# bdina9/qat-vit

Hardware: AMD Instinct MI355X
Metric: images/sec QAT student step (fwd+bwd+allreduce) (higher is better)
Workload: dtype f32 (emulated: int8 MFMA for grid x grid products; forward float operands as fp16 hi+lo pairs; backward gradients as ONE fp16 plane scaled per tensor - 2^-12 per element, <= 4e-4 relative L2 per stage against the fp32 reference, bf16-pair fallback on overflow; fp32 / exact-integer accumulate)

## Files before the change

### qat-vit_amd/csrc/elt.hip

```cpp
#include <stdlib.h>

#include "qv_common.h"
#include "qv_kernels.h"
#include "qv_qparams.h"

namespace qv {

typedef __bf16 bf16x4 __attribute__((ext_vector_type(4)));
typedef __bf16 bf16x8 __attribute__((ext_vector_type(8)));

struct QP { float s, inv, zp, on; };
__device__ inline QP load_qp(const float* qp) { return QP{qp[0], qp[1], qp[2], qp[3]}; }
__device__ inline float fqv(float x, const QP& q, float fqmin, float fqmax, bool& in) {
    const float t = rintf(x * q.inv) + q.zp;
    in = (t >= fqmin && t <= fqmax) || q.on == 0.f;
    const float y = (fminf(fmaxf(t, fqmin), fqmax) - q.zp) * q.s;
    return q.on != 0.f ? y : x;
}
__device__ inline float fqi(float x, const QP& q, float fqmin, float fqmax) {
    return fminf(fmaxf(rintf(x * q.inv) + q.zp, fqmin), fqmax) - q.zp;
}

__device__ inline void store_split4(__bf16* hi, __bf16* lo, int64_t off, float a, float b, float c, float d) {
    uint2 h, l;
    split_pair(a, b, h.x, l.x);
    split_pair(c, d, h.y, l.y);
    *reinterpret_cast<uint2*>(hi + off) = h;
    *reinterpret_cast<uint2*>(lo + off) = l;
}

__device__ inline void store_f16x4(__bf16* plane, int64_t off, float a, float b, float c, float d, float mul, float& am) {
    am = fmaxf(fmaxf(am, fmaxf(fabsf(a), fabsf(b))), fmaxf(fabsf(c), fabsf(d)));
    *reinterpret_cast<uint2*>(plane + off) = make_uint2(pk_f16(a * mul, b * mul), pk_f16(c * mul, d * mul));
}
__device__ inline void amax_publish(uint32_t* amax, float am, int lane) {
    am = wave_max(am);
    if (lane == 0) atomicMax(amax + (blockIdx.x & (kDyAmaxSlots - 1)) * kDyAmaxStride, __builtin_bit_cast(uint32_t, am));
}

static inline int rows_grid(int64_t rows) {
    int64_t b = (rows + 3) / 4;
    return (int)(b < 1 ? 1 : (b > 2048 ? 2048 : b));
}
static inline int flat_grid(int64_t n4) {
    int64_t b = (n4 + 255) / 256;
    return (int)(b < 1 ? 1 : (b > 4096 ? 4096 : b));
}

__global__ __launch_bounds__(256) void k_img_patches(const float* __restrict__ img, __bf16* __restrict__ out, const float* __restrict__ qp,
                                                     int qmin, int qmax, int B, int C, int H, int W, int P, int8_t* __restrict__ out8, int center) {
    const QP q = load_qp(qp);
    const int gw = W / P, gh = H / P, K = C * P * P;
    const int64_t n8 = (int64_t)B * gh * gw * K / 8;
    for (int64_t e8 = blockIdx.x * (int64_t)blockDim.x + threadIdx.x; e8 < n8; e8 += (int64_t)gridDim.x * blockDim.x) {
        const int64_t e = e8 * 8;
        const int col = (int)(e % K);
        const int64_t prow = e / K;
        const int px = (int)(prow % gw), py = (int)((prow / gw) % gh), b = (int)(prow / ((int64_t)gw * gh));
        const int j = col % P, i = (col / P) % P, c = col / (P * P);
        const float* src = img + (((int64_t)b * C + c) * H + py * P + i) * W + px * P + j;
        const float4 a = reinterpret_cast<const float4*>(src)[0], bb = reinterpret_cast<const float4*>(src)[1];
        bf16x8 o;
        o[0] = (__bf16)fqi(a.x, q, qmin, qmax); o[1] = (__bf16)fqi(a.y, q, qmin, qmax);
        o[2] = (__bf16)fqi(a.z, q, qmin, qmax); o[3] = (__bf16)fqi(a.w, q, qmin, qmax);
        o[4] = (__bf16)fqi(bb.x, q, qmin, qmax); o[5] = (__bf16)fqi(bb.y, q, qmin, qmax);
        o[6] = (__bf16)fqi(bb.z, q, qmin, qmax); o[7] = (__bf16)fqi(bb.w, q, qmin, qmax);
        if (out) *reinterpret_cast<bf16x8*>(out + e) = o;
        if (out8) {
            const float sh = q.zp - (float)center;
            signed char c8[8];
#pragma unroll
            for (int t = 0; t < 8; ++t) c8[t] = (signed char)((float)o[t] + sh);
            uint2 pk;
            __builtin_memcpy(&pk, c8, 8);
            *reinterpret_cast<uint2*>(out8 + e) = pk;
        }
    }
}

constexpr int kMaxV = 3;
__device__ inline void pin4(float4& v) { asm volatile("" : "+v"(v.x), "+v"(v.y), "+v"(v.z), "+v"(v.w)); }
template <int MODE, int NV>
__global__ __launch_bounds__(256) void k_resid_fq_lnstats(const float* __restrict__ x_prev, const float* __restrict__ Y, const float* __restrict__ qpY,
                                                          int qmin, int qmax, const float* __restrict__ cls, const float* __restrict__ pos,
                                                          float* __restrict__ x_new, float* __restrict__ mean, float* __restrict__ rstd,
                                                          const float* __restrict__ gamma, const float* __restrict__ beta, float eps,
                                                          uint32_t* __restrict__ stats, int stat_slots, int64_t M, int D, int T,
                                                          unsigned long long* __restrict__ maskbits, const QpLate late) {
    __shared__ float sQp[4];
    QP q;
    if (late.stats) { const float4 r = qp_late_resolve(late, sQp); q = QP{r.x, r.y, r.z, r.w}; }
    else q = load_qp(qpY);
    const int lane = threadIdx.x & 63;
    bool act[NV];
    int cc[NV];
    float4 g[NV], bb[NV];
#pragma unroll
    for (int j = 0; j < NV; ++j) {
        const int c = lane * 4 + 256 * j;
        act[j] = c < D;
        cc[j] = act[j] ? c : 0;
        g[j] = *reinterpret_cast<const float4*>(gamma + cc[j]);
        bb[j] = *reinterpret_cast<const float4*>(beta + cc[j]);
    }
    float mn = INFINITY, mx = -INFINITY;
    for (int64_t row = (int64_t)blockIdx.x * 4 + (threadIdx.x >> 6); row < M; row += (int64_t)gridDim.x * 4) {
        const int t = (int)(row % T);
        const int64_t b = row / T;
        const bool is_cls = MODE == 0 && t == 0;
        const float* bsrc = MODE == 0 ? pos + (int64_t)t * D : x_prev + row * D;
        const float* ysrc = MODE == 0 ? (is_cls ? cls : Y + (b * (T - 1) + (t - 1)) * D) : MODE == 1 ? Y + row * D : bsrc;
        float4 yr[NV], base[NV], v[NV];
#pragma unroll
        for (int j = 0; j < NV; ++j) {
            base[j] = *reinterpret_cast<const float4*>(bsrc + cc[j]);
            yr[j] = *reinterpret_cast<const float4*>(ysrc + cc[j]);
        }
#pragma unroll
        for (int j = 0; j < NV; ++j) { pin4(base[j]); pin4(yr[j]); }
        float s = 0.f;
        unsigned long long mb[NV][4];
#pragma unroll
        for (int j = 0; j < NV; ++j) {
            bool i0, i1, i2, i3;
            float4 y = make_float4(fqv(yr[j].x, q, qmin, qmax, i0), fqv(yr[j].y, q, qmin, qmax, i1), fqv(yr[j].z, q, qmin, qmax, i2),
                                   fqv(yr[j].w, q, qmin, qmax, i3));
            if (is_cls) y = yr[j];
            if (MODE == 2) y = make_float4(0.f, 0.f, 0.f, 0.f);
            if (MODE == 1) {
                mb[j][0] = __ballot(act[j] && i0); mb[j][1] = __ballot(act[j] && i1);
                mb[j][2] = __ballot(act[j] && i2); mb[j][3] = __ballot(act[j] && i3);
            }
            v[j] = make_float4(base[j].x + y.x, base[j].y + y.y, base[j].z + y.z, base[j].w + y.w);
            if (act[j]) s += (v[j].x + v[j].y) + (v[j].z + v[j].w);
        }
#pragma unroll
        for (int j = 0; j < NV; ++j)
            if (MODE != 2 && act[j]) *reinterpret_cast<float4*>(x_new + row * D + cc[j]) = v[j];
        const float mu = wave_sum(s) / (float)D;
        float qq = 0.f;
#pragma unroll
        for (int j = 0; j < NV; ++j) {
            v[j].x -= mu; v[j].y -= mu; v[j].z -= mu; v[j].w -= mu;
            if (act[j]) qq += (v[j].x * v[j].x + v[j].y * v[j].y) + (v[j].z * v[j].z + v[j].w * v[j].w);
        }
        const float rs = rsqrtf(wave_sum(qq) / (float)D + eps);
        if (lane == 0) { mean[row] = mu; rstd[row] = rs; }
        if (MODE == 1 && maskbits && lane < 4) {
#pragma unroll
            for (int j = 0; j < NV; ++j)
                maskbits[(row * NV + j) * 4 + lane] = lane == 0 ? mb[j][0] : lane == 1 ? mb[j][1] : lane == 2 ? mb[j][2] : mb[j][3];
        }
#pragma unroll
        for (int j = 0; j < NV; ++j) {
            if (act[j]) {
                const float o0 = v[j].x * rs * g[j].x + bb[j].x, o1 = v[j].y * rs * g[j].y + bb[j].y, o2 = v[j].z * rs * g[j].z + bb[j].z,
                            o3 = v[j].w * rs * g[j].w + bb[j].w;
                mn = fminf(fminf(mn, o0), fminf(o1, fminf(o2, o3)));
                mx = fmaxf(fmaxf(mx, o0), fmaxf(o1, fmaxf(o2, o3)));
            }
        }
    }
    mn = wave_min(mn);
    mx = wave_max(mx);
    __shared__ float smn[4], smx[4];
    if (lane == 0) { smn[threadIdx.x >> 6] = mn; smx[threadIdx.x >> 6] = mx; }
    __syncthreads();
    const float bmn = fminf(fminf(smn[0], smn[1]), fminf(smn[2], smn[3])), bmx = fmaxf(fmaxf(smx[0], smx[1]), fmaxf(smx[2], smx[3]));
    if (threadIdx.x == 0) stat_atomic(stats, stat_slots, bmn, bmx);
}

__global__ __launch_bounds__(256) void k_ln_apply_quant(const float* __restrict__ x, const float* __restrict__ mean, const float* __restrict__ rstd,
                                                        const float* __restrict__ gamma, const float* __restrict__ beta, const float* __restrict__ qp,
                                                        int qmin, int qmax, __bf16* __restrict__ out, int64_t M, int D,
                                                        int8_t* __restrict__ out8, int center, int out_f16, const QpLate late) {
    __shared__ float sQp[4];
    QP q;
    if (late.stats) { const float4 r = qp_late_resolve(late, sQp); q = QP{r.x, r.y, r.z, r.w}; }
    else q = load_qp(qp);
    const int d4 = D / 4;
    const int64_t n4 = M * d4;
    for (int64_t i = blockIdx.x * (int64_t)blockDim.x + threadIdx.x; i < n4; i += (int64_t)gridDim.x * blockDim.x) {
        const int64_t row = i / d4;
        const int c = (int)(i % d4) * 4;
        const float mu = mean[row], rs = rstd[row];
        const float4 v = *reinterpret_cast<const float4*>(x + row * D + c);
        const float4 g = *reinterpret_cast<const float4*>(gamma + c), b = *reinterpret_cast<const float4*>(beta + c);
        bf16x4 o;
        o[0] = (__bf16)fqi((v.x - mu) * rs * g.x + b.x, q, qmin, qmax);
        o[1] = (__bf16)fqi((v.y - mu) * rs * g.y + b.y, q, qmin, qmax);
        o[2] = (__bf16)fqi((v.z - mu) * rs * g.z + b.z, q, qmin, qmax);
        o[3] = (__bf16)fqi((v.w - mu) * rs * g.w + b.w, q, qmin, qmax);
        if (out && out_f16) *reinterpret_cast<uint2*>(out + row * D + c) = make_uint2(pk_f16((float)o[0], (float)o[1]), pk_f16((float)o[2], (float)o[3]));
        else if (out) *reinterpret_cast<bf16x4*>(out + row * D + c) = o;
        if (out8) {
            const float sh = q.zp - (float)center;
            char4 o8 = make_char4((signed char)((float)o[0] + sh), (signed char)((float)o[1] + sh), (signed char)((float)o[2] + sh),
                                  (signed char)((float)o[3] + sh));
            *reinterpret_cast<char4*>(out8 + row * D + c) = o8;
        }
    }
}

template <int NV>
__global__ __launch_bounds__(256) void k_ln_quant8(const float* __restrict__ x, const float* __restrict__ gamma, const float* __restrict__ beta, float eps,
                                                   const float* __restrict__ qp, int qmin, int qmax, int center, int8_t* __restrict__ out8,
                                                   float* __restrict__ mean, float* __restrict__ rstd, int64_t nrows, int64_t row_stride, int D) {
    const QP q = load_qp(qp);
    const int lane = threadIdx.x & 63;
    bool act[NV];
    int cc[NV];
    float4 g[NV], bb[NV];
#pragma unroll
    for (int j = 0; j < NV; ++j) {
        const int c = lane * 4 + 256 * j;
        act[j] = c < D;
        cc[j] = act[j] ? c : 0;
        g[j] = *reinterpret_cast<const float4*>(gamma + cc[j]);
        bb[j] = *reinterpret_cast<const float4*>(beta + cc[j]);
    }
    const float sh = q.zp - (float)center;
    for (int64_t i = (int64_t)blockIdx.x * 4 + (threadIdx.x >> 6); i < nrows; i += (int64_t)gridDim.x * 4) {
        const int64_t row = i * row_stride;
        float4 v[NV];
#pragma unroll
        for (int j = 0; j < NV; ++j) v[j] = *reinterpret_cast<const float4*>(x + row * D + cc[j]);
#pragma unroll
        for (int j = 0; j < NV; ++j) pin4(v[j]);
        float s = 0.f;
#pragma unroll
        for (int j = 0; j < NV; ++j)
            if (act[j]) s += (v[j].x + v[j].y) + (v[j].z + v[j].w);
        const float mu = wave_sum(s) / (float)D;
        float qq = 0.f;
        float4 cv[NV];
#pragma unroll
        for (int j = 0; j < NV; ++j) {
            cv[j] = make_float4(v[j].x - mu, v[j].y - mu, v[j].z - mu, v[j].w - mu);
            if (act[j]) qq += (cv[j].x * cv[j].x + cv[j].y * cv[j].y) + (cv[j].z * cv[j].z + cv[j].w * cv[j].w);
        }
        const float rs = rsqrtf(wave_sum(qq) / (float)D + eps);
        if (mean && lane == 0) { mean[row] = mu; rstd[row] = rs; }
        if (out8) {
#pragma unroll
            for (int j = 0; j < NV; ++j) {
                if (act[j]) {
                    const char4 o = make_char4((signed char)(fqi(cv[j].x * rs * g[j].x + bb[j].x, q, qmin, qmax) + sh),
                                               (signed char)(fqi(cv[j].y * rs * g[j].y + bb[j].y, q, qmin, qmax) + sh),
                                               (signed char)(fqi(cv[j].z * rs * g[j].z + bb[j].z, q, qmin, qmax) + sh),
                                               (signed char)(fqi(cv[j].w * rs * g[j].w + bb[j].w, q, qmin, qmax) + sh));
                    *reinterpret_cast<char4*>(out8 + row * D + cc[j]) = o;
                }
            }
        }
    }
}

__global__ __launch_bounds__(256) void k_cls_rows(const float* __restrict__ cls, const float* __restrict__ pos, float* __restrict__ x, int B, int T, int D) {
    const int64_t n = (int64_t)B * D;
    for (int64_t i = blockIdx.x * (int64_t)blockDim.x + threadIdx.x; i < n; i += (int64_t)gridDim.x * blockDim.x) {
        const int b = (int)(i / D), c = (int)(i % D);
        x[(int64_t)b * T * D + c] = cls[c] + pos[c];
    }
}

__device__ inline float gelu(float x) { return gelu_fwd(x); }
__device__ inline float dgelu(float x) { return gelu_bwd(x); }

template <int GELU_BWD, bool O16 = false>
__global__ __launch_bounds__(256) void k_mask_bwd(const float* __restrict__ d, const float* __restrict__ Y, const float* __restrict__ qp,
                                                  int qmin, int qmax, const float* __restrict__ col_scale, int ncols4,
                                                  __bf16* __restrict__ dst_hi, __bf16* __restrict__ dst_lo, int64_t n4,
                                                  const float* __restrict__ o16_mul, uint32_t* __restrict__ o16_amax) {
    const QP q = load_qp(qp);
    float mul = 1.f, am = 0.f;
    if constexpr (O16) mul = *o16_mul;
    for (int64_t i = blockIdx.x * (int64_t)blockDim.x + threadIdx.x; i < n4; i += (int64_t)gridDim.x * blockDim.x) {
        const float4 v = reinterpret_cast<const float4*>(Y)[i];
        const float4 g = reinterpret_cast<const float4*>(d)[i];
        const float in4[4] = {v.x, v.y, v.z, v.w}, g4[4] = {g.x, g.y, g.z, g.w};
        float cs[4] = {1.f, 1.f, 1.f, 1.f};
        if (col_scale) {
            const float4 c = reinterpret_cast<const float4*>(col_scale)[i % ncols4];
// ... 263 lines not shown
        if (t == 0) *reinterpret_cast<float4*>(dcls + c) = acc;
    }
}

__device__ inline void wquant_body(const float* __restrict__ W, const float* __restrict__ qp, int per_channel, int qmin, int qmax,
                                   __bf16* __restrict__ wq, __bf16* __restrict__ wqT, int N, int K, int bx, int by,
                                   int8_t* __restrict__ w8 = nullptr, int32_t* __restrict__ wsum = nullptr, _Float16* __restrict__ w16 = nullptr,
                                   int8_t* __restrict__ w8f = nullptr, int64_t wT16_gap = 0,
                                   bool wT16_frag = false) {
    __shared__ float tile[32][33];
    const int tx = threadIdx.x & 31, ty = threadIdx.x >> 5;
    const int n0 = by * 32, k0 = bx * 32;
#pragma unroll
    for (int i = 0; i < 4; ++i) {
        const int n = n0 + ty + 8 * i, k = k0 + tx;
        float v = 0.f;
        if (n < N && k < K) {
            const QP q = load_qp(qp + 4 * (per_channel ? n : 0));
            v = q.on != 0.f ? fqi(W[(int64_t)n * K + k], q, qmin, qmax) : W[(int64_t)n * K + k];
            wq[(int64_t)n * K + k] = (__bf16)v;
            if (w8) w8[(int64_t)n * K + k] = (int8_t)v;
            if (w16) w16[(int64_t)n * K + k] = (_Float16)v;
            if (w8f) w8f[w8f_offset(n, k, K)] = (int8_t)v;
        }
        tile[ty + 8 * i][tx] = v;
    }
    __syncthreads();
    if (wsum && threadIdx.x < 32 && n0 + (int)threadIdx.x < N) {
        float sacc = 0.f;
#pragma unroll
        for (int k = 0; k < 32; ++k) sacc += tile[threadIdx.x][k];
        atomicAdd(&wsum[n0 + threadIdx.x], (int)sacc);
    }
    if (wqT) {
        _Float16* const wT16 = wT16_gap ? reinterpret_cast<_Float16*>(reinterpret_cast<char*>(wqT) + wT16_gap) : nullptr;
        char* const wT16f = (wT16_gap && wT16_frag) ? reinterpret_cast<char*>(wqT) + 2 * wT16_gap : nullptr;
#pragma unroll
        for (int i = 0; i < 4; ++i) {
            const int k = k0 + ty + 8 * i, n = n0 + tx;
            if (n < N && k < K) {
                wqT[(int64_t)k * N + n] = (__bf16)tile[tx][ty + 8 * i];
                if (wT16) wT16[(int64_t)k * N + n] = (_Float16)tile[tx][ty + 8 * i];
                if (wT16f) *reinterpret_cast<_Float16*>(wT16f + w8f_offset(k, 2 * n, 2 * N)) = (_Float16)tile[tx][ty + 8 * i];
            }
        }
    }
}
__global__ __launch_bounds__(256) void k_wquant(const float* __restrict__ W, const float* __restrict__ qp, int per_channel, int qmin, int qmax,
                                                __bf16* __restrict__ wq, __bf16* __restrict__ wqT, int N, int K) {
    wquant_body(W, qp, per_channel, qmin, qmax, wq, wqT, N, K, blockIdx.x, blockIdx.y);
}
__global__ __launch_bounds__(256) void k_w_quant_all(const WQuantTab t) {
    int wi = 0;
    while (wi + 1 < t.n && (int)blockIdx.x >= t.blk0[wi + 1]) ++wi;
    const int b = blockIdx.x - t.blk0[wi], kt = (t.K[wi] + 31) / 32;
    wquant_body(t.W[wi], t.qp[wi], t.per_channel, t.qmin, t.qmax, reinterpret_cast<__bf16*>(t.wq[wi]), reinterpret_cast<__bf16*>(t.wqT[wi]), t.N[wi],
                t.K[wi], b % kt, b / kt, reinterpret_cast<int8_t*>(t.w8[wi]), t.wsum[wi], reinterpret_cast<_Float16*>(t.w16[wi]),
                reinterpret_cast<int8_t*>(t.w8f[wi]), t.wT16 ? wT16_gap_bytes(t.N[wi], t.K[wi]) : 0, ((t.wT16f_mask >> wi) & 1ull) != 0);
}
static_assert(sizeof(WQuantTab) <= 4096, "WQuantTab travels as a kernel argument");
__global__ __launch_bounds__(256) void k_w8_fragment_order(const int8_t* __restrict__ B8, int8_t* __restrict__ B8f, int N, int K) {
    const int64_t i = blockIdx.x * (int64_t)blockDim.x + threadIdx.x;
    if (i >= (int64_t)N * K) return;
    B8f[w8f_offset((int)(i / K), (int)(i % K), K)] = B8[i];
}
int launch_w8_fragment_order(const void* B8, void* B8f, int N, int K, hipStream_t st) {
    if (N < 48 || N % 48 != 0 || K % 64 != 0 || !B8 || !B8f) { set_error("w8_fragment_order: need N %% 48 == 0, K %% 64 == 0 (N=%d K=%d)", N, K); return 1; }
    k_w8_fragment_order<<<cdiv((int64_t)N * K, 256), 256, 0, st>>>(reinterpret_cast<const int8_t*>(B8), reinterpret_cast<int8_t*>(B8f), N, K);
    return 0;
}

int launch_img_patches(const float* img, void* out_bf16, const float* qp, int qmin, int qmax, int B, int C, int H, int W, int P, hipStream_t st,
                       void* out8, int center) {
    if (P % 8 != 0 || H % P != 0 || W % P != 0) { set_error("img_patches: patch %d must be a multiple of 8 and divide %dx%d", P, H, W); return 1; }
    const int64_t n8 = (int64_t)B * C * H * W / 8;
    k_img_patches<<<flat_grid(n8), 256, 0, st>>>(img, reinterpret_cast<__bf16*>(out_bf16), qp, qmin, qmax, B, C, H, W, P, reinterpret_cast<int8_t*>(out8),
                                                 center);
    return 0;
}

int launch_resid_fq_lnstats(int mode, const float* x_prev, const float* Y, const float* qpY, int qmin, int qmax, const float* cls, const float* pos,
                            float* x_new, float* mean, float* rstd, const float* gamma, const float* beta, float eps, uint32_t* stats, int stat_slots,
                            int64_t M, int D, int T, hipStream_t st, void* maskbits, const QpLate* late) {
    if (D % 4 != 0 || D > 256 * kMaxV) { set_error("resid_fq_lnstats: D=%d unsupported (need D%%4==0, D<=768)", D); return 1; }
    unsigned long long* mbits = mode != 1 ? nullptr : reinterpret_cast<unsigned long long*>(maskbits);
    const QpLate lt = late ? *late : QpLate{};
#define QV_RESID(MODE_, NV_) k_resid_fq_lnstats<MODE_, NV_><<<rows_grid(M), 256, 0, st>>>(x_prev, Y, qpY, qmin, qmax, cls, pos, x_new, mean, rstd, gamma, beta, eps, stats, stat_slots, M, D, T, mbits, lt)
    const int nv = (D + 255) / 256;
    if (mode == 0) { if (nv == 1) QV_RESID(0, 1); else if (nv == 2) QV_RESID(0, 2); else QV_RESID(0, 3); }
    else if (mode == 1) { if (nv == 1) QV_RESID(1, 1); else if (nv == 2) QV_RESID(1, 2); else QV_RESID(1, 3); }
    else { if (nv == 1) QV_RESID(2, 1); else if (nv == 2) QV_RESID(2, 2); else QV_RESID(2, 3); }
#undef QV_RESID
    return 0;
}

int launch_ln_apply_quant(const float* x, const float* mean, const float* rstd, const float* gamma, const float* beta, const float* qp, int qmin,
                          int qmax, void* out_bf16, int64_t M, int D, hipStream_t st, void* out8, int center, bool out_f16, const QpLate* late) {
    k_ln_apply_quant<<<flat_grid(M * (D / 4)), 256, 0, st>>>(x, mean, rstd, gamma, beta, qp, qmin, qmax, reinterpret_cast<__bf16*>(out_bf16), M, D,
                                                             reinterpret_cast<int8_t*>(out8), center, out_f16 ? 1 : 0, late ? *late : QpLate{});
    return 0;
}

int launch_ln_quant8(const float* x, const float* gamma, const float* beta, float eps, const float* qp, int qmin, int qmax, int center, void* out8,
                     float* mean, float* rstd, int64_t nrows, int64_t row_stride, int D, hipStream_t st) {
    if (D % 4 != 0 || D > 256 * kMaxV) { set_error("ln_quant8: D=%d unsupported (need D%%4==0, D<=768)", D); return 1; }
    const int nv = (D + 255) / 256, grid = rows_grid(nrows);
    int8_t* o = reinterpret_cast<int8_t*>(out8);
    if (nv == 1) k_ln_quant8<1><<<grid, 256, 0, st>>>(x, gamma, beta, eps, qp, qmin, qmax, center, o, mean, rstd, nrows, row_stride, D);
    else if (nv == 2) k_ln_quant8<2><<<grid, 256, 0, st>>>(x, gamma, beta, eps, qp, qmin, qmax, center, o, mean, rstd, nrows, row_stride, D);
    else k_ln_quant8<3><<<grid, 256, 0, st>>>(x, gamma, beta, eps, qp, qmin, qmax, center, o, mean, rstd, nrows, row_stride, D);
    return 0;
}
int launch_cls_rows(const float* cls, const float* pos, float* x, int B, int T, int D, hipStream_t st) {
    k_cls_rows<<<cdiv((int64_t)B * D, 256), 256, 0, st>>>(cls, pos, x, B, T, D);
    return 0;
}

int launch_mask_bwd(int gelu_bwd, const float* d, const float* Y, const float* qp, int qmin, int qmax, const float* col_scale, int ncols,
                    void* dst_hi, void* dst_lo, int64_t n, hipStream_t st, const float* o16_mul, uint32_t* o16_amax) {
    __bf16* h = reinterpret_cast<__bf16*>(dst_hi);
    __bf16* l = reinterpret_cast<__bf16*>(dst_lo);
    if (o16_mul) {
        if (gelu_bwd || !o16_amax) { set_error("mask_bwd: the one-plane form covers the plain mask with o16_amax"); return 1; }
        k_mask_bwd<0, true><<<flat_grid(n / 4), 256, 0, st>>>(d, Y, qp, qmin, qmax, col_scale, ncols / 4, h, l, n / 4, o16_mul, o16_amax);
        return 0;
    }
    if (gelu_bwd) k_mask_bwd<1><<<flat_grid(n / 4), 256, 0, st>>>(d, Y, qp, qmin, qmax, col_scale, ncols / 4, h, l, n / 4, nullptr, nullptr);
    else k_mask_bwd<0><<<flat_grid(n / 4), 256, 0, st>>>(d, Y, qp, qmin, qmax, col_scale, ncols / 4, h, l, n / 4, nullptr, nullptr);
    return 0;
}

int launch_ln_bwd_fq(int acc, const float* dH, const float* x, const float* mean, const float* rstd, const float* gamma, const float* beta,
                     const float* qp, int qmin, int qmax, const float* dx_in, float* dx_out, float* dgamma, float* dbeta, int64_t M, int D, int T,
                     int cls_only, hipStream_t st, const LnBwdNext* next) {
    if (D % 4 != 0 || D > 256 * kMaxV) { set_error("ln_bwd_fq: D=%d unsupported", D); return 1; }
    constexpr int rpw = 16;
    int grid = (int)((M + 8 * rpw - 1) / (8 * rpw));
    if (grid > 4096) grid = 4096;
    if (grid < 1) grid = 1;
    const unsigned long long* nm = next ? reinterpret_cast<const unsigned long long*>(next->maskbits) : nullptr;
    const float* ncs = next ? next->colscale : nullptr;
    __bf16* nh = next ? reinterpret_cast<__bf16*>(next->out_hi) : nullptr;
    __bf16* nl = next ? reinterpret_cast<__bf16*>(next->out_lo) : nullptr;
    const float* m16 = next ? next->o16_mul : nullptr;
    uint32_t* a16 = next ? next->o16_amax : nullptr;
    if (m16 && !a16) { set_error("ln_bwd_fq: o16_mul needs o16_amax"); return 1; }
#define QV_LNB(ACC_, NV_)                                                                                                                          \
    do {                                                                                                                                           \
        if (next && m16) k_ln_bwd_fq<ACC_, NV_, 8, true, true><<<grid, 512, 0, st>>>(dH, 0, x, mean, rstd, gamma, beta, qp, qmin, qmax, dx_in, dx_out, dgamma, dbeta, M, D, T, cls_only, nm, ncs, nh, nl, m16, a16); \
        else if (next) k_ln_bwd_fq<ACC_, NV_, 8, true><<<grid, 512, 0, st>>>(dH, 0, x, mean, rstd, gamma, beta, qp, qmin, qmax, dx_in, dx_out, dgamma, dbeta, M, D, T, cls_only, nm, ncs, nh, nl, nullptr, nullptr); \
        else k_ln_bwd_fq<ACC_, NV_, 8, false><<<grid, 512, 0, st>>>(dH, 0, x, mean, rstd, gamma, beta, qp, qmin, qmax, dx_in, dx_out, dgamma, dbeta, M, D, T, cls_only, nm, ncs, nh, nl, nullptr, nullptr); \
    } while (0)
    const int nv = (D + 255) / 256;
    if (acc) { if (nv == 1) QV_LNB(1, 1); else if (nv == 2) QV_LNB(1, 2); else QV_LNB(1, 3); }
    else { if (nv == 1) QV_LNB(0, 1); else if (nv == 2) QV_LNB(0, 2); else QV_LNB(0, 3); }
#undef QV_LNB
    return 0;
}

int launch_head_fwd(const float* x, const float* mean, const float* rstd, const float* gamma, const float* beta, const float* qp_norm, int qmin,
                    int qmax, const void* wq, const float* w_scale, int w_per_channel, const float* bias, float* hq, float* logits_pre,
                    uint32_t* stats, int stat_slots, int B, int D, int T, int C, hipStream_t st) {
    k_head_fwd<<<B, 256, D * sizeof(float), st>>>(x, mean, rstd, gamma, beta, qp_norm, qmin, qmax, reinterpret_cast<const __bf16*>(wq), w_scale,
                                                   w_per_channel, bias, hq, logits_pre, stats, stat_slots, D, T, C);
    return 0;
}

int launch_logits_fq(const float* pre, const float* qp, int qmin, int qmax, float* out, int n, hipStream_t st) {
    k_logits_fq<<<cdiv(n, 256), 256, 0, st>>>(pre, qp, qmin, qmax, out, n);
    return 0;
}

int launch_head_bwd(const float* dlogits, const float* logits_pre, const float* qp_logits, int qmin, int qmax, const float* hq, const float* qp_norm,
                    const void* wq, const float* W, const float* w_scale, const int32_t* w_zp, int w_per_channel, int w_qmin, int w_qmax, float* dW,
                    float* dbias, float* dh, int B, int D, int C, hipStream_t st) {
    k_head_bwd<<<C * ((D + 63) / 64) + B, 256, 0, st>>>(dlogits, logits_pre, qp_logits, qmin, qmax, hq, qp_norm, reinterpret_cast<const __bf16*>(wq), W, w_scale, w_zp,
                                      w_per_channel, w_qmin, w_qmax, dW, dbias, dh, B, D, C);
    return 0;
}

int launch_embed_bwd(const float* dx0, const float* Y0, const float* qp, int qmin, int qmax, float* dpos, float* dcls, void* dY0_hi, void* dY0_lo,
                     int B, int T, int D, hipStream_t st) {
// ... 30 lines not shown
```

### qat-vit_amd/csrc/engine.hip

```cpp
#include <string.h>

#include <memory>
#include <mutex>
#include <unordered_map>
#include <vector>

#include "../../include/qatvit.h"
#include <stdlib.h>

#include "qv_common.h"
#include "qv_kernels.h"

namespace qv {

enum { P_PE_W = 0, P_PE_B, P_CLS, P_POS, P_BLOCK0 };
enum { B_N1W = 0, B_N1B, B_QKVW, B_QKVB, B_PROJW, B_PROJB, B_N2W, B_N2B, B_FC1W, B_FC1B, B_FC2W, B_FC2B, B_COUNT };
enum { A_IN = 0, A_PE, A_BLOCK0 };
enum { AB_N1 = 0, AB_QKV, AB_PROJ, AB_N2, AB_FC1, AB_FC2, AB_COUNT };
enum { WB_QKV = 0, WB_PROJ, WB_FC1, WB_FC2, WB_COUNT };

struct Dims {
    int B, T, np, D, H, Hd, C, depth, Kpe, img, patch, chans;
    int64_t M;
    int n_act, n_w;
// ... 954 lines not shown
    Plan p;
    if (make_plan(*cfg, &p)) return 1;
    if (launch_dy16_set_mirror(reinterpret_cast<uint32_t*>(reinterpret_cast<char*>(workspace) + p.dy16), host_pinned, (hipStream_t)stream)) return 1;
    QV_CHECK_LAUNCH("qatvit_student_dy16_set_mirror");
    return 0;
}

int qatvit_student_dy16_to_pair(const qatvit_cfg* cfg, void* workspace, void* stream) {
    QV_CHECK_ARG(cfg && workspace, "qatvit_student_dy16_to_pair: null argument");
    if (check_cfg(*cfg)) return 1;
    Ctx x{*cfg, dims_of(*cfg), Plan(), reinterpret_cast<char*>(workspace), nullptr, nullptr, nullptr, (hipStream_t)stream, nullptr};
    if (make_plan(*cfg, &x.p)) return 1;
    for (int i = 0; i < x.d.depth; ++i) {
        if (x.p.form.x_plane_from_q8) {
            if (launch_q8_to_bf16int(x.blk<void>(x.p.h1q8, i), x.act_qp(x.aidx(i, AB_N1)), x.center(), x.blk<void>(x.p.h1q, i), x.d.M * x.d.D, x.st)) return 1;
            if (launch_q8_to_bf16int(x.blk<void>(x.p.h2q8, i), x.act_qp(x.aidx(i, AB_N2)), x.center(), x.blk<void>(x.p.h2q, i), x.d.M * x.d.D, x.st)) return 1;
            continue;
        }
        if (launch_f16int_to_bf16int(x.blk<void>(x.p.h1q, i), x.d.M * x.d.D, x.st)) return 1;
        if (launch_f16int_to_bf16int(x.blk<void>(x.p.h2q, i), x.d.M * x.d.D, x.st)) return 1;
    }
    QV_CHECK_LAUNCH("qatvit_student_dy16_to_pair");
    return 0;
}

int qatvit_profile_start(const void* workspace, int32_t kind, int32_t max_launches) {
    QV_CHECK_ARG(workspace && kind >= 1 && kind <= 9 && max_launches > 0, "qatvit_profile_start: bad arguments");
    auto pr = std::make_shared<Prof>();
    pr->ev.assign((size_t)max_launches * 2, nullptr);
    for (auto& e : pr->ev)
        if (hipEventCreate(&e) != hipSuccess) {
            set_error("qatvit_profile_start: hipEventCreate failed");
            return 2;
        }
    pr->kind = kind;
    std::lock_guard<std::mutex> lk(g_prof_mu);
    auto it = g_profs.find(workspace);
    if (it != g_profs.end()) {
        std::lock_guard<std::mutex> l2(it->second->mu);
        it->second->closed = true;
    }
    g_profs[workspace] = pr;
    return 0;
}

int qatvit_profile_stop(const void* workspace, double* total_ms, int64_t* launches, double* flops) {
    QV_CHECK_ARG(workspace && total_ms && launches && flops, "qatvit_profile_stop: null argument");
    std::shared_ptr<Prof> pr;
    {
        std::lock_guard<std::mutex> lk(g_prof_mu);
        auto it = g_profs.find(workspace);
        if (it != g_profs.end()) { pr = it->second; g_profs.erase(it); }
    }
    QV_CHECK_ARG(pr, "qatvit_profile_stop: no profile is active for this workspace");
    size_t used;
    {
        std::lock_guard<std::mutex> lk(pr->mu);
        pr->closed = true;
        used = pr->used;
        *flops = pr->flops;
    }
    double ms = 0.0;
    for (size_t i = 0; i + 1 < used; i += 2) {
        if (hipEventSynchronize(pr->ev[i + 1]) != hipSuccess) continue;
        float t = 0.f;
        if (hipEventElapsedTime(&t, pr->ev[i], pr->ev[i + 1]) == hipSuccess) ms += t;
    }
    *total_ms = ms;
    *launches = (int64_t)(used / 2);
    return 0;
}

int64_t qatvit_student_tensor_offset(const qatvit_cfg* cfg, const char* name, int32_t block) {
    if (!cfg || !name || check_cfg(*cfg)) return -1;
    Plan p;
    if (make_plan(*cfg, &p)) return -1;
    struct { const char* n; int64_t off; bool per_block; } tab[] = {
        {"Y0", p.Y0, false}, {"imgq", p.imgq, false}, {"hq", p.hq, false}, {"logits_pre", p.logits_pre, false}, {"x_in", p.x_in, true},
        {"x_mid", p.x_mid, true}, {"h1q", p.h1q, true}, {"qkv", p.qkv, true}, {"O_hi", p.O_hi, true}, {"O_lo", p.O_lo, true}, {"Yproj", p.Yproj, true}, {"h2q", p.h2q, true},
        {"Y1", p.Y1, true}, {"G_hi", p.G_hi, true}, {"G_lo", p.G_lo, true}, {"Y2", p.Y2, true}, {"dxA", p.dxA, false}, {"dqkv_hi", p.dqkv_hi, false},
        {"dqkv_lo", p.dqkv_lo, false}, {"dO", p.dO, false},
        {"dH", p.dH, false}, {"lse", p.lse, true}, {"O16_hi", p.O16_hi, true}, {"O16_lo", p.O16_lo, true}, {"G16_hi", p.G16_hi, false},
        {"G16_lo", p.G16_lo, false}, {"scal16", p.scal16, true}, {"dy16", p.dy16, false}, {"dYs_hi", p.dYs_hi, false}, {"dY1_hi", p.dY1_hi, false}, {"G8", p.G8, true}, {"glut", p.glut, true}, {"Y1m", p.Y1m, true}, {"glutq", p.glutq, true}, {"qkv8", p.qkv8, true}, {"qkvm", p.qkvm, true},
    };
    for (auto& t : tab)
        if (strcmp(t.n, name) == 0) return t.off + (t.per_block ? p.blk_stride * block : 0);
    return -1;
}

}
```

Before: 16090.

## Restructure residual-LN and LN-apply kernels with half-wave rows and load prefetch

Rewrites the residual+fake-quant+LN-stats kernel so a wave can handle two rows with half-waves when D is not a multiple of 256 at 512 or above, and software-prefetches the next row's operands while processing the current one. The LN apply/quant kernel becomes row-oriented with 8-wide vectors, per-lane gamma/beta kept in registers, and the same prefetch. Both kernels get an occupancy-sized persistent grid from a cached occupancy query. This targets idle lanes at D=384-like widths and exposed memory latency, at the cost of more registers, tighter D constraints (D%128==0), and a rewritten mask-bit layout for the half-wave case. It also exposes extra tensor offsets for debugging.

```diff
diff --git a/qat-vit_amd/csrc/elt.hip b/qat-vit_amd/csrc/elt.hip
--- a/qat-vit_amd/csrc/elt.hip
+++ b/qat-vit_amd/csrc/elt.hip
@@ -1,4 +1,8 @@
 #include <stdlib.h>
+
+#include <mutex>
+#include <utility>
+#include <vector>
 
 #include "qv_common.h"
 #include "qv_kernels.h"
@@ -80,86 +84,151 @@
 
 constexpr int kMaxV = 3;
 __device__ inline void pin4(float4& v) { asm volatile("" : "+v"(v.x), "+v"(v.y), "+v"(v.z), "+v"(v.w)); }
-template <int MODE, int NV>
-__global__ __launch_bounds__(256) void k_resid_fq_lnstats(const float* __restrict__ x_prev, const float* __restrict__ Y, const float* __restrict__ qpY,
-                                                          int qmin, int qmax, const float* __restrict__ cls, const float* __restrict__ pos,
-                                                          float* __restrict__ x_new, float* __restrict__ mean, float* __restrict__ rstd,
-                                                          const float* __restrict__ gamma, const float* __restrict__ beta, float eps,
-                                                          uint32_t* __restrict__ stats, int stat_slots, int64_t M, int D, int T,
-                                                          unsigned long long* __restrict__ maskbits, const QpLate late) {
+__device__ inline float half_wave_sum(float v) {
+#pragma unroll
+    for (int o = 16; o > 0; o >>= 1) v += __shfl_xor(v, o, 64);
+    return v;
+}
+
+static int row_kernel_cus() {
+    static int cus = 0;
+    if (!cus) {
+        int dev = 0;
+        if (hipGetDevice(&dev) != hipSuccess || hipDeviceGetAttribute(&cus, hipDeviceAttributeMultiprocessorCount, dev) != hipSuccess || cus < 1 || cus > 1024) cus = 256;
+    }
+    return cus;
+}
+static int row_kernel_occupancy(const void* kernel) {
+    static std::mutex mu;
+    static std::vector<std::pair<const void*, int>> seen;
+    std::lock_guard<std::mutex> g(mu);
+    for (auto& s : seen)
+        if (s.first == kernel) return s.second;
+    int n = 0;
+    if (hipOccupancyMaxActiveBlocksPerMultiprocessor(&n, kernel, 256, 0) != hipSuccess || n < 1) n = 1;
+    seen.emplace_back(kernel, n);
+    return n;
+}
+static int row_kernel_grid(const void* kernel, int64_t units) {
+    const int64_t cap = (int64_t)row_kernel_cus() * row_kernel_occupancy(kernel) * 4;
+    const int64_t rounds = units > cap ? (units + cap - 1) / cap : 1;
+    const int64_t waves = (units + rounds - 1) / rounds;
+    return (int)((waves + 3) / 4 > 0 ? (waves + 3) / 4 : 1);
+}
+
+template <int MODE, int HALF, int G>
+__global__ __launch_bounds__(256, G > 3 ? 2 : 4) void k_resid_fq_lnstats(const float* __restrict__ x_prev, const float* __restrict__ Y, const float* __restrict__ qpY,
+                                                             int qmin, int qmax, const float* __restrict__ cls, const float* __restrict__ pos,
+                                                             float* __restrict__ x_new, float* __restrict__ mean, float* __restrict__ rstd,
+                                                             const float* __restrict__ gamma, const float* __restrict__ beta, float eps,
+                                                             uint32_t* __restrict__ stats, int stat_slots, int64_t M, int D, int T,
+                                                             unsigned long long* __restrict__ maskbits, const QpLate late) {
+    constexpr int RPU = HALF ? 2 : 1, CSTEP = HALF ? 128 : 256, NV = HALF ? (G + 1) / 2 : G;
+    const int lane = threadIdx.x & 63, h = HALF ? lane & 31 : lane;
+    const int64_t gw = (int64_t)blockIdx.x * 4 + (threadIdx.x >> 6), W = (int64_t)gridDim.x * 4, units = (M + RPU - 1) / RPU;
+    int cc[G];
+#pragma unroll
+    for (int k = 0; k < G; ++k) cc[k] = 4 * h + CSTEP * k;
+    auto load = [&](int64_t u, float4 (&base)[G], float4 (&yr)[G]) {
+        int64_t row = u * RPU + (HALF ? lane >> 5 : 0);
+        if (row >= M) row = M - 1;
+        const float* bsrc = x_prev + row * D;
+        const float* ysrc = Y + row * D;
+        if (MODE == 0) {
+            const int t = (int)row % T, b = (int)row / T;
+            bsrc = pos + (int64_t)t * D;
+            ysrc = t == 0 ? cls : Y + ((int64_t)b * (T - 1) + (t - 1)) * D;
+        }
+#pragma unroll
+        for (int k = 0; k < G; ++k) {
+            base[k] = *reinterpret_cast<const float4*>(bsrc + cc[k]);
+            yr[k] = MODE == 2 ? make_float4(0.f, 0.f, 0.f, 0.f) : *reinterpret_cast<const float4*>(ysrc + cc[k]);
+        }
+    };
+    float4 cb[G], cy[G];
+    load(gw, cb, cy);
     __shared__ float sQp[4];
     QP q;
     if (late.stats) { const float4 r = qp_late_resolve(late, sQp); q = QP{r.x, r.y, r.z, r.w}; }
     else q = load_qp(qpY);
-    const int lane = threadIdx.x & 63;
-    bool act[NV];
-    int cc[NV];
-    float4 g[NV], bb[NV];
-#pragma unroll
-    for (int j = 0; j < NV; ++j) {
-        const int c = lane * 4 + 256 * j;
-        act[j] = c < D;
-        cc[j] = act[j] ? c : 0;
-        g[j] = *reinterpret_cast<const float4*>(gamma + cc[j]);
-        bb[j] = *reinterpret_cast<const float4*>(beta + cc[j]);
+    float4 g[G], bb[G];
+#pragma unroll
+    for (int k = 0; k < G; ++k) {
+        g[k] = *reinterpret_cast<const float4*>(gamma + cc[k]);
+        bb[k] = *reinterpret_cast<const float4*>(beta + cc[k]);
     }
     float mn = INFINITY, mx = -INFINITY;
-    for (int64_t row = (int64_t)blockIdx.x * 4 + (threadIdx.x >> 6); row < M; row += (int64_t)gridDim.x * 4) {
-        const int t = (int)(row % T);
-        const int64_t b = row / T;
-        const bool is_cls = MODE == 0 && t == 0;
-        const float* bsrc = MODE == 0 ? pos + (int64_t)t * D : x_prev + row * D;
-        const float* ysrc = MODE == 0 ? (is_cls ? cls : Y + (b * (T - 1) + (t - 1)) * D) : MODE == 1 ? Y + row * D : bsrc;
-        float4 yr[NV], base[NV], v[NV];
-#pragma unroll
-        for (int j = 0; j < NV; ++j) {
-            base[j] = *reinterpret_cast<const float4*>(bsrc + cc[j]);
-            yr[j] = *reinterpret_cast<const float4*>(ysrc + cc[j]);
-        }
-#pragma unroll
-        for (int j = 0; j < NV; ++j) { pin4(base[j]); pin4(yr[j]); }
-        float s = 0.f;
-        unsigned long long mb[NV][4];
-#pragma unroll
-        for (int j = 0; j < NV; ++j) {
+    auto process = [&](int64_t u, float4 (&cb)[G], float4 (&cy)[G]) {
+        const int64_t row0 = u * RPU + (HALF ? lane >> 5 : 0);
+        const bool live = row0 < M;
+        const int64_t row = live ? row0 : M - 1;
+        const bool is_cls = MODE == 0 && (int)row % T == 0;
+        float4 v[G];
+        unsigned long long mb[G][4];
+        float sa = 0.f, sb = 0.f;
+#pragma unroll
+        for (int k = 0; k < G; ++k) {
             bool i0, i1, i2, i3;
-            float4 y = make_float4(fqv(yr[j].x, q, qmin, qmax, i0), fqv(yr[j].y, q, qmin, qmax, i1), fqv(yr[j].z, q, qmin, qmax, i2),
-                                   fqv(yr[j].w, q, qmin, qmax, i3));
-            if (is_cls) y = yr[j];
+            float4 y = make_float4(fqv(cy[k].x, q, qmin, qmax, i0), fqv(cy[k].y, q, qmin, qmax, i1), fqv(cy[k].z, q, qmin, qmax, i2),
+                                   fqv(cy[k].w, q, qmin, qmax, i3));
+            if (is_cls) y = cy[k];
             if (MODE == 2) y = make_float4(0.f, 0.f, 0.f, 0.f);
             if (MODE == 1) {
-                mb[j][0] = __ballot(act[j] && i0); mb[j][1] = __ballot(act[j] && i1);
-                mb[j][2] = __ballot(act[j] && i2); mb[j][3] = __ballot(act[j] && i3);
-            }
-            v[j] = make_float4(base[j].x + y.x, base[j].y + y.y, base[j].z + y.z, base[j].w + y.w);
-            if (act[j]) s += (v[j].x + v[j].y) + (v[j].z + v[j].w);
-        }
-#pragma unroll
-        for (int j = 0; j < NV; ++j)
-            if (MODE != 2 && act[j]) *reinterpret_cast<float4*>(x_new + row * D + cc[j]) = v[j];
-        const float mu = wave_sum(s) / (float)D;
-        float qq = 0.f;
-#pragma unroll
-        for (int j = 0; j < NV; ++j) {
-            v[j].x -= mu; v[j].y -= mu; v[j].z -= mu; v[j].w -= mu;
-            if (act[j]) qq += (v[j].x * v[j].x + v[j].y * v[j].y) + (v[j].z * v[j].z + v[j].w * v[j].w);
-        }
-        const float rs = rsqrtf(wave_sum(qq) / (float)D + eps);
-        if (lane == 0) { mean[row] = mu; rstd[row] = rs; }
-        if (MODE == 1 && maskbits && lane < 4) {
-#pragma unroll
-            for (int j = 0; j < NV; ++j)
-                maskbits[(row * NV + j) * 4 + lane] = lane == 0 ? mb[j][0] : lane == 1 ? mb[j][1] : lane == 2 ? mb[j][2] : mb[j][3];
-        }
-#pragma unroll
-        for (int j = 0; j < NV; ++j) {
-            if (act[j]) {
-                const float o0 = v[j].x * rs * g[j].x + bb[j].x, o1 = v[j].y * rs * g[j].y + bb[j].y, o2 = v[j].z * rs * g[j].z + bb[j].z,
-                            o3 = v[j].w * rs * g[j].w + bb[j].w;
+                mb[k][0] = __ballot(i0); mb[k][1] = __ballot(i1); mb[k][2] = __ballot(i2); mb[k][3] = __ballot(i3);
+            }
+            v[k] = make_float4(cb[k].x + y.x, cb[k].y + y.y, cb[k].z + y.z, cb[k].w + y.w);
+            const float p = (v[k].x + v[k].y) + (v[k].z + v[k].w);
+            if (HALF && (k & 1)) sb += p; else sa += p;
+        }
+#pragma unroll
+        for (int k = 0; k < G; ++k)
+            if (MODE != 2 && live) *reinterpret_cast<float4*>(x_new + row * D + cc[k]) = v[k];
+        const float mu = (HALF ? half_wave_sum(sa + sb) : wave_sum(sa)) / (float)D;
+        float qa = 0.f, qb = 0.f;
+#pragma unroll
+        for (int k = 0; k < G; ++k) {
+            v[k].x -= mu; v[k].y -= mu; v[k].z -= mu; v[k].w -= mu;
+            const float p = (v[k].x * v[k].x + v[k].y * v[k].y) + (v[k].z * v[k].z + v[k].w * v[k].w);
+            if (HALF && (k & 1)) qb += p; else qa += p;
+        }
+        const float rs = rsqrtf((HALF ? half_wave_sum(qa + qb) : wave_sum(qa)) / (float)D + eps);
+        if (live && h == 0) { mean[row] = mu; rstd[row] = rs; }
+        if (MODE == 1 && maskbits) {
+            constexpr int WPR = NV * 4;
+            const int r = lane / WPR, j = (lane / 4) % NV, e = lane & 3;
+            unsigned long long w = 0;
+#pragma unroll
+            for (int jj = 0; jj < NV; ++jj)
+#pragma unroll
+                for (int ee = 0; ee < 4; ++ee) {
+                    if (HALF) {
+                        const unsigned long long lo = mb[2 * jj][ee], hi = 2 * jj + 1 < G ? mb[2 * jj + 1 < G ? 2 * jj + 1 : 0][ee] : 0ull;
+                        const unsigned long long w0 = (lo & 0xffffffffull) | (hi << 32), w1 = (lo >> 32) | (hi & 0xffffffff00000000ull);
+                        if (j == jj && e == ee) w = r == 0 ? w0 : w1;
+                    } else if (j == jj && e == ee) {
+                        w = mb[jj][ee];
+                    }
+                }
+            const int64_t wrow = u * RPU + r;
+            if (lane < RPU * WPR && wrow < M) maskbits[wrow * WPR + lane % WPR] = w;
+        }
+        if (live) {
+#pragma unroll
+            for (int k = 0; k < G; ++k) {
+                const float o0 = v[k].x * rs * g[k].x + bb[k].x, o1 = v[k].y * rs * g[k].y + bb[k].y, o2 = v[k].z * rs * g[k].z + bb[k].z,
+                            o3 = v[k].w * rs * g[k].w + bb[k].w;
                 mn = fminf(fminf(mn, o0), fminf(o1, fminf(o2, o3)));
                 mx = fmaxf(fmaxf(mx, o0), fmaxf(o1, fmaxf(o2, o3)));
             }
         }
+    };
+    for (int64_t u = gw; u < units; u += W) {
+        float4 nb[G], ny[G];
+        if (u + W < units) load(u + W, nb, ny);
+        asm volatile("" ::: "memory");
+        process(u, cb, cy);
+#pragma unroll
+        for (int k = 0; k < G; ++k) { cb[k] = nb[k]; cy[k] = ny[k]; }
     }
     mn = wave_min(mn);
     mx = wave_max(mx);
@@ -170,35 +239,83 @@
     if (threadIdx.x == 0) stat_atomic(stats, stat_slots, bmn, bmx);
 }
 
-__global__ __launch_bounds__(256) void k_ln_apply_quant(const float* __restrict__ x, const float* __restrict__ mean, const float* __restrict__ rstd,
-                                                        const float* __restrict__ gamma, const float* __restrict__ beta, const float* __restrict__ qp,
-                                                        int qmin, int qmax, __bf16* __restrict__ out, int64_t M, int D,
-                                                        int8_t* __restrict__ out8, int center, int out_f16, const QpLate late) {
+template <int LPR, int C>
+__global__ __launch_bounds__(256, C > 3 ? 2 : 4) void k_ln_apply_quant(const float* __restrict__ x, const float* __restrict__ mean, const float* __restrict__ rstd,
+                                                           const float* __restrict__ gamma, const float* __restrict__ beta, const float* __restrict__ qp,
+                                                           int qmin, int qmax, __bf16* __restrict__ out, int64_t M, int D,
+                                                           int8_t* __restrict__ out8, int center, int out_f16, const QpLate late) {
+    constexpr int RPU = 64 / LPR, CSTEP = 8 * LPR;
+    const int lane = threadIdx.x & 63, h = lane % LPR;
+    const int64_t gw = (int64_t)blockIdx.x * 4 + (threadIdx.x >> 6), W = (int64_t)gridDim.x * 4, units = (M + RPU - 1) / RPU;
+    int cc[C];
+#pragma unroll
+    for (int k = 0; k < C; ++k) cc[k] = 8 * h + CSTEP * k;
+    auto load = [&](int64_t u, float4 (&v)[2 * C], float& mu, float& rs) {
+        int64_t row = u * RPU + lane / LPR;
+        if (row >= M) row = M - 1;
+        mu = mean[row];
+        rs = rstd[row];
+#pragma unroll
+        for (int k = 0; k < C; ++k) {
+            v[2 * k] = *reinterpret_cast<const float4*>(x + row * D + cc[k]);
+            v[2 * k + 1] = *reinterpret_cast<const float4*>(x + row * D + cc[k] + 4);
+        }
+    };
+    float4 cv[2 * C];
+    float cmu, crs;
+    load(gw, cv, cmu, crs);
     __shared__ float sQp[4];
     QP q;
     if (late.stats) { const float4 r = qp_late_resolve(late, sQp); q = QP{r.x, r.y, r.z, r.w}; }
     else q = load_qp(qp);
-    const int d4 = D / 4;
-    const int64_t n4 = M * d4;
-    for (int64_t i = blockIdx.x * (int64_t)blockDim.x + threadIdx.x; i < n4; i += (int64_t)gridDim.x * blockDim.x) {
-        const int64_t row = i / d4;
-        const int c = (int)(i % d4) * 4;
-        const float mu = mean[row], rs = rstd[row];
-        const float4 v = *reinterpret_cast<const float4*>(x + row * D + c);
-        const float4 g = *reinterpret_cast<const float4*>(gamma + c), b = *reinterpret_cast<const float4*>(beta + c);
-        bf16x4 o;
-        o[0] = (__bf16)fqi((v.x - mu) * rs * g.x + b.x, q, qmin, qmax);
-        o[1] = (__bf16)fqi((v.y - mu) * rs * g.y + b.y, q, qmin, qmax);
-        o[2] = (__bf16)fqi((v.z - mu) * rs * g.z + b.z, q, qmin, qmax);
-        o[3] = (__bf16)fqi((v.w - mu) * rs * g.w + b.w, q, qmin, qmax);
-        if (out && out_f16) *reinterpret_cast<uint2*>(out + row * D + c) = make_uint2(pk_f16((float)o[0], (float)o[1]), pk_f16((float)o[2], (float)o[3]));
-        else if (out) *reinterpret_cast<bf16x4*>(out + row * D + c) = o;
-        if (out8) {
-            const float sh = q.zp - (float)center;
-            char4 o8 = make_char4((signed char)((float)o[0] + sh), (signed char)((float)o[1] + sh), (signed char)((float)o[2] + sh),
-                                  (signed char)((float)o[3] + sh));
-            *reinterpret_cast<char4*>(out8 + row * D + c) = o8;
-        }
+    float4 g[2 * C], bb[2 * C];
+#pragma unroll
+    for (int k = 0; k < 2 * C; ++k) {
+        g[k] = *reinterpret_cast<const float4*>(gamma + cc[k / 2] + 4 * (k & 1));
+        bb[k] = *reinterpret_cast<const float4*>(beta + cc[k / 2] + 4 * (k & 1));
+    }
+    const float sh = q.zp - (float)center;
+    auto process = [&](int64_t u, const float4 (&cv)[2 * C], float mu, float rs) {
+        const int64_t row = u * RPU + lane / LPR;
+        if (row < M) {
+#pragma unroll
+            for (int k = 0; k < C; ++k) {
+                const float4 a = cv[2 * k], b = cv[2 * k + 1], ga = g[2 * k], gb = g[2 * k + 1], ba = bb[2 * k], bt = bb[2 * k + 1];
+                bf16x8 o;
+                o[0] = (__bf16)fqi((a.x - mu) * rs * ga.x + ba.x, q, qmin, qmax);
+                o[1] = (__bf16)fqi((a.y - mu) * rs * ga.y + ba.y, q, qmin, qmax);
+                o[2] = (__bf16)fqi((a.z - mu) * rs * ga.z + ba.z, q, qmin, qmax);
+                o[3] = (__bf16)fqi((a.w - mu) * rs * ga.w + ba.w, q, qmin, qmax);
+                o[4] = (__bf16)fqi((b.x - mu) * rs * gb.x + bt.x, q, qmin, qmax);
+                o[5] = (__bf16)fqi((b.y - mu) * rs * gb.y + bt.y, q, qmin, qmax);
+                o[6] = (__bf16)fqi((b.z - mu) * rs * gb.z + bt.z, q, qmin, qmax);
+                o[7] = (__bf16)fqi((b.w - mu) * rs * gb.w + bt.w, q, qmin, qmax);
+                const int64_t off = row * D + cc[k];
+                if (out && out_f16)
+                    *reinterpret_cast<uint4*>(out + off) = make_uint4(pk_f16((float)o[0], (float)o[1]), pk_f16((float)o[2], (float)o[3]),
+                                                                      pk_f16((float)o[4], (float)o[5]), pk_f16((float)o[6], (float)o[7]));
+                else if (out) *reinterpret_cast<bf16x8*>(out + off) = o;
+                if (out8) {
+                    signed char c8[8];
+#pragma unroll
+                    for (int t = 0; t < 8; ++t) c8[t] = (signed char)((float)o[t] + sh);
+                    uint2 pk;
+                    __builtin_memcpy(&pk, c8, 8);
+                    *reinterpret_cast<uint2*>(out8 + off) = pk;
+                }
+            }
+        }
+    };
+    for (int64_t u = gw; u < units; u += W) {
+        float4 nv[2 * C];
+        float nmu, nrs;
+        if (u + W < units) load(u + W, nv, nmu, nrs);
+        asm volatile("" ::: "memory");
+        process(u, cv, cmu, crs);
+#pragma unroll
+        for (int k = 0; k < 2 * C; ++k) cv[k] = nv[k];
+        cmu = nmu;
+        crs = nrs;
     }
 }
 
@@ -628,22 +745,56 @@
 int launch_resid_fq_lnstats(int mode, const float* x_prev, const float* Y, const float* qpY, int qmin, int qmax, const float* cls, const float* pos,
                             float* x_new, float* mean, float* rstd, const float* gamma, const float* beta, float eps, uint32_t* stats, int stat_slots,
                             int64_t M, int D, int T, hipStream_t st, void* maskbits, const QpLate* late) {
-    if (D % 4 != 0 || D > 256 * kMaxV) { set_error("resid_fq_lnstats: D=%d unsupported (need D%%4==0, D<=768)", D); return 1; }
+    if (D % 128 != 0 || D > 768 || mode < 0 || mode > 2 || M < 1 || M > INT32_MAX) {
+        set_error("resid_fq_lnstats: D=%d M=%lld mode %d unsupported (need D %% 128 == 0, D <= 768)", D, (long long)M, mode);
+        return 1;
+    }
     unsigned long long* mbits = mode != 1 ? nullptr : reinterpret_cast<unsigned long long*>(maskbits);
     const QpLate lt = late ? *late : QpLate{};
-#define QV_RESID(MODE_, NV_) k_resid_fq_lnstats<MODE_, NV_><<<rows_grid(M), 256, 0, st>>>(x_prev, Y, qpY, qmin, qmax, cls, pos, x_new, mean, rstd, gamma, beta, eps, stats, stat_slots, M, D, T, mbits, lt)
-    const int nv = (D + 255) / 256;
-    if (mode == 0) { if (nv == 1) QV_RESID(0, 1); else if (nv == 2) QV_RESID(0, 2); else QV_RESID(0, 3); }
-    else if (mode == 1) { if (nv == 1) QV_RESID(1, 1); else if (nv == 2) QV_RESID(1, 2); else QV_RESID(1, 3); }
-    else { if (nv == 1) QV_RESID(2, 1); else if (nv == 2) QV_RESID(2, 2); else QV_RESID(2, 3); }
+    const bool half = !(D % 256 == 0 && D >= 512);
+    const int g = half ? D / 128 : D / 256;
+    const int64_t units = half ? (M + 1) / 2 : M;
+#define QV_RESID(MODE_, HALF_, G_)                                                                                                                     \
+    do {                                                                                                                                               \
+        auto k = &k_resid_fq_lnstats<MODE_, HALF_, G_>;                                                                                                \
+        k<<<row_kernel_grid(reinterpret_cast<const void*>(k), units), 256, 0, st>>>(x_prev, Y, qpY, qmin, qmax, cls, pos, x_new, mean, rstd, gamma,    \
+                                                                                    beta, eps, stats, stat_slots, M, D, T, mbits, lt);                  \
+    } while (0)
+#define QV_RESID_G(MODE_)                                                                                                                              \
+    do {                                                                                                                                               \
+        if (!half) { if (g == 2) QV_RESID(MODE_, 0, 2); else QV_RESID(MODE_, 0, 3); }                                                                 \
+        else if (g == 1) QV_RESID(MODE_, 1, 1);                                                                                                        \
+        else if (g == 2) QV_RESID(MODE_, 1, 2);                                                                                                        \
+        else if (g == 3) QV_RESID(MODE_, 1, 3);                                                                                                        \
+        else QV_RESID(MODE_, 1, 5);                                                                                                                    \
+    } while (0)
+    if (mode == 0) QV_RESID_G(0);
+    else if (mode == 1) QV_RESID_G(1);
+    else QV_RESID_G(2);
+#undef QV_RESID_G
 #undef QV_RESID
     return 0;
 }
 
 int launch_ln_apply_quant(const float* x, const float* mean, const float* rstd, const float* gamma, const float* beta, const float* qp, int qmin,
                           int qmax, void* out_bf16, int64_t M, int D, hipStream_t st, void* out8, int center, bool out_f16, const QpLate* late) {
-    k_ln_apply_quant<<<flat_grid(M * (D / 4)), 256, 0, st>>>(x, mean, rstd, gamma, beta, qp, qmin, qmax, reinterpret_cast<__bf16*>(out_bf16), M, D,
-                                                             reinterpret_cast<int8_t*>(out8), center, out_f16 ? 1 : 0, late ? *late : QpLate{});
+    if (D % 128 != 0 || D > 768 || M < 1) { set_error("ln_apply_quant: D=%d unsupported (need D %% 128 == 0, D <= 768)", D); return 1; }
+    const int n = D / 128;
+    const QpLate lt = late ? *late : QpLate{};
+#define QV_LNQ(LPR_, C_)                                                                                                                               \
+    do {                                                                                                                                               \
+        auto k = &k_ln_apply_quant<LPR_, C_>;                                                                                                          \
+        k<<<row_kernel_grid(reinterpret_cast<const void*>(k), (M + 64 / LPR_ - 1) / (64 / LPR_)), 256, 0, st>>>(                                       \
+            x, mean, rstd, gamma, beta, qp, qmin, qmax, reinterpret_cast<__bf16*>(out_bf16), M, D, reinterpret_cast<int8_t*>(out8), center,            \
+            out_f16 ? 1 : 0, lt);                                                                                                                      \
+    } while (0)
+    if (n == 1) QV_LNQ(16, 1);
+    else if (n == 2) QV_LNQ(16, 2);
+    else if (n == 3) QV_LNQ(16, 3);
+    else if (n == 4) QV_LNQ(32, 2);
+    else if (n == 5) QV_LNQ(16, 5);
+    else QV_LNQ(32, 3);
+#undef QV_LNQ
     return 0;
 }
 
diff --git a/qat-vit_amd/csrc/engine.hip b/qat-vit_amd/csrc/engine.hip
--- a/qat-vit_amd/csrc/engine.hip
+++ b/qat-vit_amd/csrc/engine.hip
@@ -1060,6 +1060,8 @@
         {"dqkv_lo", p.dqkv_lo, false}, {"dO", p.dO, false},
         {"dH", p.dH, false}, {"lse", p.lse, true}, {"O16_hi", p.O16_hi, true}, {"O16_lo", p.O16_lo, true}, {"G16_hi", p.G16_hi, false},
         {"G16_lo", p.G16_lo, false}, {"scal16", p.scal16, true}, {"dy16", p.dy16, false}, {"dYs_hi", p.dYs_hi, false}, {"dY1_hi", p.dY1_hi, false}, {"G8", p.G8, true}, {"glut", p.glut, true}, {"Y1m", p.Y1m, true}, {"glutq", p.glutq, true}, {"qkv8", p.qkv8, true}, {"qkvm", p.qkvm, true},
+        {"mean1", p.mean1, true}, {"rstd1", p.rstd1, true}, {"mean2", p.mean2, true}, {"rstd2", p.rstd2, true}, {"mproj", p.mproj, true}, {"m2", p.m2, true},
+        {"h1q8", p.h1q8, true}, {"h2q8", p.h2q8, true}, {"meanF", p.meanF, false}, {"rstdF", p.rstdF, false},
     };
     for (auto& t : tab)
         if (strcmp(t.n, name) == 0) return t.off + (t.per_block ? p.blk_stride * block : 0);
```

Result: no change. 16230 (median of 6 runs) (+0.9%).
